# chintha/U-VIP-SLAM

Measured on AMD Instinct MI355X. Metric: frames/sec ORB extract+match, 640x512 @1000 kp, higher is better.
Workload: dtype u8; 1 GPU; BASELINE.json configs[2]: 1xMI355X per rank, batch=256 synthetic 640x512 mono frames (+1 halo frame: the neighbouring rank's first), 1000 feats, 8 levels, fastTh 20, FullDetect extract + all-pairs 256-bit Hamming knn-2 of consecutive frames, HBM-resident I/O; batch_per_gpu=256, pipeline_depth=2, input_batches_in_rotation=4, fast_mode=adaptive

## Files before the change

### u-vip-slam_amd/csrc/hamming.hip

```cpp
#include "common.hpp"

namespace uvo {

constexpr int HM_TILE = 128;

__device__ __forceinline__ int popc256(const uint4& qa, const uint4& qb, const uint4& ta, const uint4& tb) {
  int d = __popc(qa.x ^ ta.x);
  d += __popc(qa.y ^ ta.y);
  d += __popc(qa.z ^ ta.z);
  d += __popc(qa.w ^ ta.w);
  d += __popc(qb.x ^ tb.x);
  d += __popc(qb.y ^ tb.y);
  d += __popc(qb.z ^ tb.z);
  d += __popc(qb.w ^ tb.w);
  return d;
}

__device__ __forceinline__ int clamp_count(int n, int cap) { return n < 0 ? 0 : (n > cap ? cap : n); }

__global__ __launch_bounds__(256) void k_knn2(const uint8_t* __restrict__ q, const int32_t* __restrict__ nq_arr, int nq_fixed, int q_stride,
                                              const uint8_t* __restrict__ t, const int32_t* __restrict__ nt_arr, int nt_fixed, int t_stride,
                                              const uint8_t* __restrict__ mask, int out_stride, int32_t* __restrict__ idx0,
                                              uint16_t* __restrict__ d0, int32_t* __restrict__ idx1, uint16_t* __restrict__ d1) {
  __shared__ uint4 s_t[HM_TILE * 2];
  const int pair = blockIdx.y;
  const int nq = nq_arr ? clamp_count(nq_arr[pair], q_stride < out_stride ? q_stride : out_stride) : nq_fixed;
  const int nt = nt_arr ? clamp_count(nt_arr[pair], t_stride < 65535 ? t_stride : 65535) : nt_fixed;
  const int qi = blockIdx.x * 256 + threadIdx.x;
  if (blockIdx.x * 256 >= nq) return;
  const uint4* Q = reinterpret_cast<const uint4*>(q + (int64_t)pair * q_stride * 32);
  const uint4* T = reinterpret_cast<const uint4*>(t + (int64_t)pair * t_stride * 32);
  const bool live = qi < nq;
  uint4 qa = make_uint4(0, 0, 0, 0), qb = qa;
  if (live) {
    qa = Q[2 * qi];
    qb = Q[2 * qi + 1];
  }
  uint32_t k0 = 0xFFFFFFFFu, k1 = 0xFFFFFFFFu;
  const uint8_t* mrow = mask ? mask + (int64_t)qi * nt : nullptr;
  for (int base = 0; base < nt; base += HM_TILE) {
    const int cnt = nt - base < HM_TILE ? nt - base : HM_TILE;
    __syncthreads();
    if ((int)threadIdx.x < 2 * cnt) s_t[threadIdx.x] = T[2 * base + threadIdx.x];
    __syncthreads();
    if (live) {
      for (int j = 0; j < cnt; ++j) {
        const uint32_t d = (uint32_t)popc256(qa, qb, s_t[2 * j], s_t[2 * j + 1]);
        uint32_t key = (d << 16) | (uint32_t)(base + j);
        if (mrow && !mrow[base + j]) key = 0xFFFFFFFFu;
        const uint32_t lo = min(k0, key);
        k1 = min(k1, max(k0, key));
        k0 = lo;
      }
    }
  }
  if (live) {
    const int64_t o = (int64_t)pair * out_stride + qi;
    idx0[o] = k0 == 0xFFFFFFFFu ? -1 : (int32_t)(k0 & 0xffffu);
    d0[o] = k0 == 0xFFFFFFFFu ? (uint16_t)0xFFFF : (uint16_t)(k0 >> 16);
    idx1[o] = k1 == 0xFFFFFFFFu ? -1 : (int32_t)(k1 & 0xffffu);
    d1[o] = k1 == 0xFFFFFFFFu ? (uint16_t)0xFFFF : (uint16_t)(k1 >> 16);
  }
}

typedef int v4i __attribute__((ext_vector_type(4)));
typedef int v16i __attribute__((ext_vector_type(16)));
constexpr int KM_ROW = 272;

__device__ __forceinline__ uint32_t spread4(uint32_t t) { return (__umul24(t & 0xfu, 0x00204081u)) & 0x01010101u; }
__device__ __forceinline__ v4i spread16(uint32_t x) {
  v4i r;
  r.x = (int)spread4(x), r.y = (int)spread4(x >> 4), r.z = (int)spread4(x >> 8), r.w = (int)spread4(x >> 12);
  return r;
}
__device__ __forceinline__ uint32_t spread4_ff(uint32_t t) {
  const uint32_t b = spread4(t);
  return (b << 8) - b;
}
__device__ __forceinline__ v4i spread16_ff(uint32_t x) {
  v4i r;
  r.x = (int)spread4_ff(x), r.y = (int)spread4_ff(x >> 4), r.z = (int)spread4_ff(x >> 8), r.w = (int)spread4_ff(x >> 12);
  return r;
}

__device__ __forceinline__ int med3_i32(int a, int b, int c) {
  int r;
  asm("v_med3_i32 %0, %1, %2, %3" : "=v"(r) : "v"(a), "v"(b), "v"(c));
  return r;
}

#ifndef UVO_OCC_KNN
#define UVO_OCC_KNN 6
#endif
__global__ __launch_bounds__(256, UVO_OCC_KNN) void k_knn2_mfma(const uint8_t* __restrict__ q, const int32_t* __restrict__ nq_arr, int nq_fixed, int q_stride,
                                                   const uint8_t* __restrict__ t, const int32_t* __restrict__ nt_arr, int nt_fixed, int t_stride,
                                                   int out_stride, int32_t* __restrict__ idx0, uint16_t* __restrict__ d0,
                                                   int32_t* __restrict__ idx1, uint16_t* __restrict__ d1) {
  __shared__ __attribute__((aligned(16))) uint8_t s_exp[32 * KM_ROW];
  __shared__ __attribute__((aligned(16))) int32_t s_key[32];
  const int pair = blockIdx.y;
  const int nq = nq_arr ? clamp_count(nq_arr[pair], q_stride < out_stride ? q_stride : out_stride) : nq_fixed;
  const int nt = nt_arr ? clamp_count(nt_arr[pair], t_stride < 65535 ? t_stride : 65535) : nt_fixed;
  if (blockIdx.x * 128 >= nq) return;
  const int lane = threadIdx.x & 63, wv = wave_in_block();
  const int r = lane & 31, h = lane >> 5;
  const int qi = blockIdx.x * 128 + wv * 32 + r;
  const uint32_t* Q = reinterpret_cast<const uint32_t*>(q + (int64_t)pair * q_stride * 32);
  const uint32_t* T = reinterpret_cast<const uint32_t*>(t + (int64_t)pair * t_stride * 32);
  v4i bq[8];
  int popq = 0;
#pragma unroll
  for (int s = 0; s < 8; ++s) {
    const uint32_t w = qi < nq ? Q[(int64_t)qi * 8 + s] : 0u;
    popq += __popc(w);
    bq[s] = spread16_ff(w >> (16 * h));
  }
  int k0 = 0x7fffffff, k1 = 0x7fffffff;
  const int erow = threadIdx.x >> 3, ec = threadIdx.x & 7;
  uint32_t wnext = erow < nt ? T[(int64_t)erow * 8 + ec] : 0u;
  for (int base = 0; base < nt; base += 32) {
    __syncthreads();
    {
      const int tr = base + erow;
      const uint32_t w = wnext;
      wnext = tr + 32 < nt ? T[(int64_t)(tr + 32) * 8 + ec] : 0u;
      v4i* dst = reinterpret_cast<v4i*>(s_exp + erow * KM_ROW + ec * 32);
      dst[0] = spread16(w), dst[1] = spread16(w >> 16);
      int pc = __popc(w);
      pc += __shfl_xor(pc, 1, 64);
      pc += __shfl_xor(pc, 2, 64);
      pc += __shfl_xor(pc, 4, 64);
      if (ec == 0) s_key[erow] = tr < nt ? ((pc << 16) | tr) : 0x7fff0000;
    }
    __syncthreads();
    v16i acc = {0, 0, 0, 0, 0, 0, 0, 0, 0, 0, 0, 0, 0, 0, 0, 0};
    const uint8_t* arow = s_exp + r * KM_ROW + 16 * h;
#pragma unroll
    for (int s = 0; s < 8; ++s) {
      const v4i a = *reinterpret_cast<const v4i*>(arow + 32 * s);
      acc = __builtin_amdgcn_mfma_i32_32x32x32_i8(a, bq[s], acc, 0, 0, 0);
    }
#pragma unroll
    for (int g = 0; g < 4; ++g) {
      const v4i kb = *reinterpret_cast<const v4i*>(&s_key[8 * g + 4 * h]);
      const int kbv[4] = {kb.x, kb.y, kb.z, kb.w};
#pragma unroll
      for (int e = 0; e < 4; ++e) {
        const int key = (int)(((uint32_t)acc[4 * g + e] << 17) + (uint32_t)kbv[e]);
        k1 = med3_i32(k0, k1, key);
        k0 = min(k0, key);
      }
    }
  }
  const int o0 = __shfl_xor(k0, 32, 64), o1 = __shfl_xor(k1, 32, 64);
  const int m0 = min(k0, o0), m1 = min(max(k0, o0), min(k1, o1));
  if (h == 0 && qi < nq) {
    const int64_t o = (int64_t)pair * out_stride + qi;
    const bool v0 = m0 < 0x7fff0000, v1 = m1 < 0x7fff0000;
    idx0[o] = v0 ? (m0 & 0xffff) : -1;
    d0[o] = v0 ? (uint16_t)((m0 >> 16) + popq) : (uint16_t)0xFFFF;
    idx1[o] = v1 ? (m1 & 0xffff) : -1;
    d1[o] = v1 ? (uint16_t)((m1 >> 16) + popq) : (uint16_t)0xFFFF;
  }
}

__global__ __launch_bounds__(256) void k_matrix(const uint8_t* __restrict__ q, int nq, const uint8_t* __restrict__ t, int nt,
                                                uint16_t* __restrict__ dist) {
  __shared__ uint4 s_t[HM_TILE * 2];
  const int qi = blockIdx.x * 256 + threadIdx.x;
  const uint4* Q = reinterpret_cast<const uint4*>(q);
  const uint4* T = reinterpret_cast<const uint4*>(t);
  const bool live = qi < nq;
  uint4 qa = make_uint4(0, 0, 0, 0), qb = qa;
  if (live) {
    qa = Q[2 * qi];
    qb = Q[2 * qi + 1];
  }
  const int base = blockIdx.y * HM_TILE;
  const int cnt = nt - base < HM_TILE ? nt - base : HM_TILE;
  if ((int)threadIdx.x < 2 * cnt) s_t[threadIdx.x] = T[2 * base + threadIdx.x];
  __syncthreads();
  if (!live) return;
  for (int j = 0; j < cnt; ++j) dist[(int64_t)qi * nt + base + j] = (uint16_t)popc256(qa, qb, s_t[2 * j], s_t[2 * j + 1]);
}

__global__ __launch_bounds__(256) void k_medoid(const uint8_t* __restrict__ desc, const int32_t* __restrict__ offsets, int32_t* __restrict__ best_idx,
                                                int32_t* __restrict__ best_median) {
  __shared__ uint32_t s_best;
  const int p = blockIdx.x;
  const int o0 = offsets[p], n = offsets[p + 1] - o0;
  if (threadIdx.x == 0) s_best = 0xFFFFFFFFu;
  __syncthreads();
  if (n > 0) {
    const uint4* D = reinterpret_cast<const uint4*>(desc + (int64_t)o0 * 32);
    const int k = (int)(0.5 * (n - 1));
    for (int i = threadIdx.x; i < n; i += 256) {
      const uint4 qa = D[2 * i], qb = D[2 * i + 1];
      int lo = 0, hi = 256;
      while (lo < hi) {
        const int mid = (lo + hi) >> 1;
        int c = 0;
        for (int j = 0; j < n; ++j) c += popc256(qa, qb, D[2 * j], D[2 * j + 1]) <= mid;
        if (c >= k + 1)
          hi = mid;
        else
          lo = mid + 1;
      }
      atomicMin(&s_best, ((uint32_t)lo << 16) | (uint32_t)i);
    }
  }
  __syncthreads();
  if (threadIdx.x == 0) {
    best_idx[p] = n > 0 ? (int32_t)(s_best & 0xffffu) : -1;
    best_median[p] = n > 0 ? (int32_t)(s_best >> 16) : -1;
  }
}

void launch_medoid(hipStream_t s, const uint8_t* d_desc, const int32_t* d_offsets, int npoints, int32_t* d_idx, int32_t* d_med) {
  hipLaunchKernelGGL(k_medoid, dim3(npoints), dim3(256), 0, s, d_desc, d_offsets, d_idx, d_med);
}

void launch_knn2(hipStream_t s, int pairs, int max_q, const uint8_t* d_q, const int32_t* d_nq, int nq_fixed, int q_stride, const uint8_t* d_t,
                 const int32_t* d_nt, int nt_fixed, int t_stride, const uint8_t* d_mask, int out_stride, int32_t* d_idx0, uint16_t* d_d0,
                 int32_t* d_idx1, uint16_t* d_d1) {
  if (!d_mask) {
    hipLaunchKernelGGL(k_knn2_mfma, dim3((max_q + 127) / 128, pairs), dim3(256), 0, s, d_q, d_nq, nq_fixed, q_stride, d_t, d_nt, nt_fixed, t_stride,
                       out_stride, d_idx0, d_d0, d_idx1, d_d1);
    return;
  }
  hipLaunchKernelGGL(k_knn2, dim3((max_q + 255) / 256, pairs), dim3(256), 0, s, d_q, d_nq, nq_fixed, q_stride, d_t, d_nt, nt_fixed, t_stride,
                     d_mask, out_stride, d_idx0, d_d0, d_idx1, d_d1);
}

void launch_matrix(hipStream_t s, const uint8_t* d_q, int nq, const uint8_t* d_t, int nt, uint16_t* d_dist) {
  hipLaunchKernelGGL(k_matrix, dim3((nq + 255) / 256, (nt + HM_TILE - 1) / HM_TILE), dim3(256), 0, s, d_q, nq, d_t, nt, d_dist);
}

}
```

### u-vip-slam_amd/csrc/tune_internal.h

```cpp
#pragma once
#define UVO_TUNE_PYR_RING 12
#define UVO_TUNE_FUSE_BLUR_TREE 10
#define UVO_TUNE_PYR_FORM 13
#define UVO_PYR_FORM_AUTO 0
#define UVO_PYR_FORM_LEVELS 1
#define UVO_PYR_FORM_TILES 2
#define UVO_PYR_FORM_ROWS 3
#define UVO_TUNE_PYR_TILE_GROUP 14
#define UVO_TUNE_FEW_FRAMES 16
#define UVO_TUNE_ZERO_COPY_OUT 17
#define UVO_TUNE_SPIN_WAIT 18
```

### u-vip-slam_amd/csrc/gauss_body.hpp

```cpp
#pragma once
#include "common.hpp"
#include "fast_geom.hpp"
#include <type_traits>

namespace uvo {

typedef unsigned short u16x2 __attribute__((ext_vector_type(2)));
__device__ __forceinline__ u16x2 pk(uint32_t x) { return __builtin_bit_cast(u16x2, x); }

struct GaussRowTaps {
  uint32_t l0, c0, l1, c1, r1, l2, c2, r2, c3, r3;
};
__device__ __forceinline__ GaussRowTaps gauss_row_taps(int4 t) {
  auto pk4 = [](int a, int b, int c, int d) { return (uint32_t)a | ((uint32_t)b << 8) | ((uint32_t)c << 16) | ((uint32_t)d << 24); };
  GaussRowTaps T;
  T.l0 = pk4(0, t.x, t.y, t.z), T.c0 = pk4(t.w, t.z, t.y, t.x);
  T.l1 = pk4(0, 0, t.x, t.y), T.c1 = pk4(t.z, t.w, t.z, t.y), T.r1 = pk4(t.x, 0, 0, 0);
  T.l2 = pk4(0, 0, 0, t.x), T.c2 = pk4(t.y, t.z, t.w, t.z), T.r2 = pk4(t.y, t.x, 0, 0);
  T.c3 = pk4(t.x, t.y, t.z, t.w), T.r3 = pk4(t.z, t.y, t.x, 0);
  return T;
}
__device__ __forceinline__ void gauss_row_pass(uint32_t L, uint32_t C, uint32_t R, const GaussRowTaps& T, float* h) {
  const uint32_t s0 = __builtin_amdgcn_udot4(C, T.c0, __builtin_amdgcn_udot4(L, T.l0, 0u, false), false);
  const uint32_t s1 = __builtin_amdgcn_udot4(R, T.r1, __builtin_amdgcn_udot4(C, T.c1, __builtin_amdgcn_udot4(L, T.l1, 0u, false), false), false);
  const uint32_t s2 = __builtin_amdgcn_udot4(R, T.r2, __builtin_amdgcn_udot4(C, T.c2, __builtin_amdgcn_udot4(L, T.l2, 0u, false), false), false);
  const uint32_t s3 = __builtin_amdgcn_udot4(R, T.r3, __builtin_amdgcn_udot4(C, T.c3, 0u, false), false);
  h[0] = (float)s0, h[1] = (float)s1, h[2] = (float)s2, h[3] = (float)s3;
}

struct GaussPlans {
  StripPlan p[kMaxLevels];
};
int gauss7_rows_per_seg(int batch);
int gauss7_blocks_per_frame(const Geom& g, int rows_per_seg);
GaussPlans gauss7_plans(const Geom& g, int rows_per_seg);
constexpr int GS_TILES = 16;
constexpr int GS_TILE_DW = GS_TILES * 32 + 96;
constexpr int GS_LDS_BYTES = 4 * GS_TILE_DW * 4;
template <bool SSE2>
__device__ __forceinline__ void gauss7_body(int block, int blocks_x, int batch, uint32_t (*s_tile)[GS_TILE_DW], const uint8_t* __restrict__ pyr,
                                            uint8_t* __restrict__ blur, int64_t pyr_block, const LevelGeom* __restrict__ lv, int nlevels, int4 taps, int rows_per_seg,
                                            Level0View l0, const GaussPlans& plans) {
  const int vb = xcd_contiguous(block, blocks_x * batch);
  const int vbx = vb % blocks_x, f = vb / blocks_x;
  int item = vbx * 4 + wave_in_block();
  const int lane = threadIdx.x & 63;
  int level = 0;
  for (;; ++level) {
    if (item < plans.p[level].items) break;
    item -= plans.p[level].items;
    if (level == nlevels - 1) return;
  }
  const StripPlan plan = plans.p[level];
  const LevelGeom g = lv[level];
  int strip_x, seg, nsub;
  fast_strip_item(plan, item, strip_x, seg, nsub);
  auto walk = [&](auto ip_tag, auto tail_tag) {
  constexpr bool IP = decltype(ip_tag)::value;
  constexpr bool TAIL = decltype(tail_tag)::value;
  const uint8_t* src = IP ? l0.vbase + f * l0.frame_stride + (int64_t)kPad * l0.pitch + kPad : pyr + f * pyr_block + g.plane_off;
  const int spitch = IP ? l0.pitch : g.pitch;
  uint8_t* dst = blur + f * pyr_block + g.plane_off;

  const int lps = 64 / nsub, sub = (lane * nsub) >> 6, ls = lane - sub * lps;
  const int X = 8 + strip_x + ls * 4;
  int Xc = X > g.pitch - 4 ? g.pitch - 4 : X;
  uint32_t csel = 0x03020100u;
  if (IP) {
    const int x = X - kPad;
    int run = x;
    if (x < 0) run = -x - 3, csel = 0x00010203u;
    else if (x > g.w - 4) run = 2 * (g.w - 1) - x - 3, csel = 0x00010203u;
    Xc = run < 0 ? 0 : (run > g.w - 4 ? g.w - 4 : run);
  }
  const int py0 = 12 + seg * rows_per_seg;
  const int py0l = py0 + sub * rows_per_seg;
  const int py1l = min(py0l + rows_per_seg, g.h + 20);
  const bool lane_out = ls >= 1 && ls <= lps - 2 && X >= 12 && X < g.w + 20 && py1l > py0l;
  const int tile_col = (X >> 4) * 128 + (X & 15);
  const int64_t tile_row_bytes = (int64_t)g.pitch * 8;
  const int x_lo = max(12, 8 + strip_x + 4), x_hi = min(g.w + 20, 8 + strip_x + 4 * (lps - 1));
  const int t_first = (x_lo + 15) >> 4, nts = max((x_hi >> 4) - t_first, 0);
  const int ts_shift = nsub == 1 ? 4 : (nsub == 2 ? 3 : 2), TS = 1 << ts_shift;
  const bool via_lds = lane_out && (X >> 4) >= t_first && (X >> 4) < t_first + nts;
  uint32_t* stile = s_tile[wave_in_block()];
  const int lds_slot = via_lds ? ((sub * TS + ((X >> 4) - t_first)) << 5) + ((X & 15) >> 2) : GS_TILES * 32 + lane;
  const int64_t seg_tile_rows = (int64_t)(rows_per_seg >> 3) * tile_row_bytes;
  const int64_t lane_goff = (int64_t)sub * seg_tile_rows + tile_col;
  int f_lds[2], f_p0[2], f_p1[2], f_rowoff[2];
  int64_t f_goff[2];
#pragma unroll
  for (int it = 0; it < 2; ++it) {
    const int t = lane + 64 * it, row = t & 7, slot = t >> 3, s_ = slot >> ts_shift, ti = slot & (TS - 1);
    const int p0 = py0 + s_ * rows_per_seg;
    f_lds[it] = (slot << 5) + (row << 2);
    f_goff[it] = (int64_t)s_ * seg_tile_rows + (t_first + ti) * 128 + (row << 4);
    f_rowoff[it] = s_ * rows_per_seg + row;
    f_p0[it] = p0, f_p1[it] = (s_ < nsub && ti < nts) ? min(p0 + rows_per_seg, g.h + 20) : p0;
  }
  auto flush_tiles = [&](int pyg, int r_hi, int64_t group_base) {
    __builtin_amdgcn_wave_barrier();
#pragma unroll
    for (int it = 0; it < 2; ++it) {
      const int prow = pyg + f_rowoff[it];
      if ((lane & 7) <= r_hi && prow >= f_p0[it] && prow < f_p1[it]) {
        const uint4 v = *reinterpret_cast<const uint4*>(stile + f_lds[it]);
        *reinterpret_cast<uint4*>(dst + (group_base + f_goff[it])) = v;
      }
    }
    __builtin_amdgcn_wave_barrier();
  };

  const bool tail_lane = SSE2 && (g.w & 3) != 0 && (X - kPad) == (g.w & ~3);
  uint32_t inmask = 0;
#pragma unroll
  for (int k = 0; k < 4; ++k) inmask |= (X + k >= kPad && X + k < g.w + kPad) ? 0xffu << (8 * k) : 0u;
  const int nsrc = min(py0 + rows_per_seg, g.h + 20) - py0 + 6;
  const uint32_t j_in0 = (uint32_t)(kPad - py0l + 6), n_in = (uint32_t)g.h;
  const uint32_t j_edge1 = (lane_out && !via_lds) ? (uint32_t)max(py1l - py0l + 6, 0) : 0u;

  const GaussRowTaps RT = gauss_row_taps(taps);
  const float c0 = (float)taps.x * (1.0f / 65536.0f), c1 = (float)taps.y * (1.0f / 65536.0f), c2 = (float)taps.z * (1.0f / 65536.0f),
              c3 = (float)taps.w * (1.0f / 65536.0f);
  if (!SSE2) __builtin_amdgcn_s_setreg(0x801, 3);
  const int lane_up = (lane > 0 ? lane - 1 : lane) * 4, lane_down = (lane < 63 ? lane + 1 : lane) * 4;
  float hring[7][4];
  uint32_t cring[7];
  auto load_row = [&](int j) -> uint32_t {
    int prow = py0l - 3 + j;
    if (IP) {
      int r = prow - kPad;
      r = r < 0 ? -r : r;
      r = r > g.h - 1 ? 2 * (g.h - 1) - r : r;
      r = r < 0 ? 0 : r;
      const uint32_t v = *reinterpret_cast<const uint32_t*>(src + (__umul24((uint32_t)r, (uint32_t)spitch) + (uint32_t)Xc));
      return __builtin_amdgcn_perm(v, v, csel);
    }
    prow = prow > g.ph - 1 ? g.ph - 1 : prow;
    return *reinterpret_cast<const uint32_t*>(src + (__umul24((uint32_t)prow, (uint32_t)spitch) + (uint32_t)Xc));
  };
  int64_t rowb = (int64_t)(py0 >> 3) * tile_row_bytes + ((py0 & 7) << 4);
  int phase = (py0 - 6) & 7;
  uint32_t cur[7], nxt[7];
#pragma unroll
  for (int u = 0; u < 7; ++u) cur[u] = load_row(u);
  for (int base = 0; base < nsrc; base += 7) {
#pragma unroll
    for (int u = 0; u < 7; ++u) nxt[u] = load_row(base + 7 + u);
#pragma unroll
    for (int u = 0; u < 7; ++u) {
      const int j = base + u;
      if (j < nsrc) {
        const uint32_t C = cur[u];
        const uint32_t L = (uint32_t)__builtin_amdgcn_ds_bpermute(lane_up, (int)C);
        const uint32_t R = (uint32_t)__builtin_amdgcn_ds_bpermute(lane_down, (int)C);
        gauss_row_pass(L, C, R, RT, hring[u]);
        cring[u] = C;
        const int phase_now = phase;
        phase = (phase + 1) & 7;
        if (j >= 6) {
          const float* r0 = hring[(u + 1) % 7];
          const float* r1 = hring[(u + 2) % 7];
          const float* r2 = hring[(u + 3) % 7];
          const float* r3 = hring[(u + 4) % 7];
          const float* r4 = hring[(u + 5) % 7];
          const float* r5 = hring[(u + 6) % 7];
          const float* r6 = hring[u];
          const uint32_t centre = cring[(u + 4) % 7];
          const bool row_in = (uint32_t)j - j_in0 < n_in;
          uint32_t blurred = 0;
#pragma unroll
          for (int k = 0; k < 4; ++k) {
            float z = __builtin_fmaf(c0, r0[k] + r6[k], __builtin_fmaf(c1, r1[k] + r5[k], __builtin_fmaf(c2, r2[k] + r4[k], __builtin_fmaf(c3, r3[k], SSE2 ? 0.0f : 0.5f))));
            if (SSE2 && TAIL) z = tail_lane ? __builtin_floorf(z + 0.5f) : z;
            blurred = __builtin_amdgcn_cvt_pk_u8_f32(z, (uint32_t)k, blurred);
          }
          const uint32_t m = row_in ? inmask : 0u;
          const uint32_t out = (blurred & m) | (centre & ~m);
          stile[lds_slot + (phase_now << 2)] = out;
          if ((uint32_t)j < j_edge1) *reinterpret_cast<uint32_t*>(dst + rowb + lane_goff) = out;
          if (phase_now == 7) {
            flush_tiles(py0 + j - 6 - 7, 7, rowb - 112);
            rowb += tile_row_bytes - 112;
          } else {
            rowb += 16;
          }
        }
      }
    }
#pragma unroll
    for (int u = 0; u < 7; ++u) cur[u] = nxt[u];
  }
  {
    const int py_last = py0 + nsrc - 7;
    if ((py_last & 7) != 7) flush_tiles(py_last & ~7, py_last & 7, (int64_t)(py_last >> 3) * tile_row_bytes);
  }
  };
  const int x_last = 8 + strip_x + 4 * (64 / nsub - 1);
  const bool tail_wave = SSE2 && (g.w & 3) != 0 && kPad + (g.w & ~3) >= 8 + strip_x && kPad + (g.w & ~3) < x_last;
  if (level == 0 && l0.vbase != nullptr)
    walk(std::true_type{}, std::false_type{});
  else if (tail_wave)
    walk(std::false_type{}, std::true_type{});
  else
    walk(std::false_type{}, std::false_type{});
}


}
```

Before: 329,300 frames/s.

## Fold train popcount and index key into MFMA accumulator init for knn2

Reworks the MFMA Hamming knn-2 kernel. When the train count fits in 12 bits, descriptor bits are pre-shifted (<<7 for queries, <<6 for train) so the int8 MFMA directly produces distance<<13 plus the (popcount<<12|index) key loaded as the accumulator init, removing the per-element shift/add. It also widens the workgroup to 8 waves (256 queries) with 64 train rows staged per sync, and uses DPP instead of shuffles for the popcount reduction. Gains are fewer VALU ops and syncs per tile, at the cost of higher register pressure, a second kernel variant for large train sets, and idle non-expander waves during staging.

```diff
diff --git a/u-vip-slam_amd/csrc/hamming.hip b/u-vip-slam_amd/csrc/hamming.hip
--- a/u-vip-slam_amd/csrc/hamming.hip
+++ b/u-vip-slam_amd/csrc/hamming.hip
@@ -1,4 +1,5 @@
 #include "common.hpp"
+#include "tune_internal.h"
 
 namespace uvo {
 
@@ -82,6 +83,25 @@
   r.x = (int)spread4_ff(x), r.y = (int)spread4_ff(x >> 4), r.z = (int)spread4_ff(x >> 8), r.w = (int)spread4_ff(x >> 12);
   return r;
 }
+template <int SH>
+__device__ __forceinline__ uint32_t spread4_at(uint32_t t) {
+  static_assert(SH + 24 < 32, "the product leaves 32 bits");
+  return (__umul24(t & (0xfu << SH), 0x00204081u)) & (0x01010101u << SH);
+}
+template <int SH>
+__device__ __forceinline__ v4i spread16_shl(uint32_t x) {
+  const uint32_t y = x << SH;
+  v4i r;
+  r.x = (int)spread4_at<SH>(y), r.y = (int)spread4_at<SH>(y >> 4), r.z = (int)spread4_at<SH>(y >> 8), r.w = (int)spread4_at<SH>(y >> 12);
+  return r;
+}
+
+__device__ __forceinline__ int sum8_dpp(int v) {
+  v += __builtin_amdgcn_update_dpp(0, v, 0xB1, 0xf, 0xf, true);
+  v += __builtin_amdgcn_update_dpp(0, v, 0x4E, 0xf, 0xf, true);
+  v += __builtin_amdgcn_update_dpp(0, v, 0x141, 0xf, 0xf, true);
+  return v;
+}
 
 __device__ __forceinline__ int med3_i32(int a, int b, int c) {
   int r;
@@ -89,22 +109,33 @@
   return r;
 }
 
-#ifndef UVO_OCC_KNN
-#define UVO_OCC_KNN 6
+#ifndef UVO_KNN_WAVES
+#define UVO_KNN_WAVES 8
 #endif
-__global__ __launch_bounds__(256, UVO_OCC_KNN) void k_knn2_mfma(const uint8_t* __restrict__ q, const int32_t* __restrict__ nq_arr, int nq_fixed, int q_stride,
-                                                   const uint8_t* __restrict__ t, const int32_t* __restrict__ nt_arr, int nt_fixed, int t_stride,
-                                                   int out_stride, int32_t* __restrict__ idx0, uint16_t* __restrict__ d0,
-                                                   int32_t* __restrict__ idx1, uint16_t* __restrict__ d1) {
-  __shared__ __attribute__((aligned(16))) uint8_t s_exp[32 * KM_ROW];
-  __shared__ __attribute__((aligned(16))) int32_t s_key[32];
+#ifndef UVO_KNN_ROWS
+#define UVO_KNN_ROWS 64
+#endif
+constexpr int KM_WAVES = UVO_KNN_WAVES, KM_QUERIES = 32 * KM_WAVES, KM_ROWS = UVO_KNN_ROWS;
+constexpr int KM_FOLD_BITS = 12, KM_FOLD_MAX_TRAIN = 1 << KM_FOLD_BITS;
+static_assert(24 % KM_WAVES == 0 && (KM_ROWS == 32 || KM_ROWS == 64) && KM_ROWS * 8 <= 64 * KM_WAVES, "workgroup shape");
+
+template <bool FOLD>
+__device__ __forceinline__ void knn2_mfma_body(const uint8_t* __restrict__ q, const int32_t* __restrict__ nq_arr, int nq_fixed, int q_stride,
+                                               const uint8_t* __restrict__ t, const int32_t* __restrict__ nt_arr, int nt_fixed, int t_stride,
+                                               int out_stride, int32_t* __restrict__ idx0, uint16_t* __restrict__ d0,
+                                               int32_t* __restrict__ idx1, uint16_t* __restrict__ d1) {
+  __shared__ __attribute__((aligned(16))) uint8_t s_exp[KM_ROWS * KM_ROW];
+  __shared__ __attribute__((aligned(16))) int32_t s_key[KM_ROWS];
+  constexpr int IDX_BITS = FOLD ? KM_FOLD_BITS : 16;
   const int pair = blockIdx.y;
   const int nq = nq_arr ? clamp_count(nq_arr[pair], q_stride < out_stride ? q_stride : out_stride) : nq_fixed;
   const int nt = nt_arr ? clamp_count(nt_arr[pair], t_stride < 65535 ? t_stride : 65535) : nt_fixed;
-  if (blockIdx.x * 128 >= nq) return;
+  if (blockIdx.x * KM_QUERIES >= nq) return;
   const int lane = threadIdx.x & 63, wv = wave_in_block();
   const int r = lane & 31, h = lane >> 5;
-  const int qi = blockIdx.x * 128 + wv * 32 + r;
+  const int qi = blockIdx.x * KM_QUERIES + wv * 32 + r;
+  const bool active = blockIdx.x * KM_QUERIES + wv * 32 < nq;
+  const bool expander = wv < KM_ROWS / 8;
   const uint32_t* Q = reinterpret_cast<const uint32_t*>(q + (int64_t)pair * q_stride * 32);
   const uint32_t* T = reinterpret_cast<const uint32_t*>(t + (int64_t)pair * t_stride * 32);
   v4i bq[8];
@@ -113,42 +144,50 @@
   for (int s = 0; s < 8; ++s) {
     const uint32_t w = qi < nq ? Q[(int64_t)qi * 8 + s] : 0u;
     popq += __popc(w);
-    bq[s] = spread16_ff(w >> (16 * h));
+    bq[s] = FOLD ? spread16_shl<7>(w >> (16 * h)) : spread16_ff(w >> (16 * h));
   }
   int k0 = 0x7fffffff, k1 = 0x7fffffff;
   const int erow = threadIdx.x >> 3, ec = threadIdx.x & 7;
-  uint32_t wnext = erow < nt ? T[(int64_t)erow * 8 + ec] : 0u;
-  for (int base = 0; base < nt; base += 32) {
+  uint32_t wnext = expander && erow < nt ? T[(int64_t)erow * 8 + ec] : 0u;
+  for (int base = 0; base < nt; base += KM_ROWS) {
     __syncthreads();
-    {
+    if (expander) {
       const int tr = base + erow;
       const uint32_t w = wnext;
-      wnext = tr + 32 < nt ? T[(int64_t)(tr + 32) * 8 + ec] : 0u;
+      wnext = tr + KM_ROWS < nt ? T[(int64_t)(tr + KM_ROWS) * 8 + ec] : 0u;
       v4i* dst = reinterpret_cast<v4i*>(s_exp + erow * KM_ROW + ec * 32);
-      dst[0] = spread16(w), dst[1] = spread16(w >> 16);
-      int pc = __popc(w);
-      pc += __shfl_xor(pc, 1, 64);
-      pc += __shfl_xor(pc, 2, 64);
-      pc += __shfl_xor(pc, 4, 64);
-      if (ec == 0) s_key[erow] = tr < nt ? ((pc << 16) | tr) : 0x7fff0000;
+      dst[0] = FOLD ? spread16_shl<6>(w) : spread16(w), dst[1] = FOLD ? spread16_shl<6>(w >> 16) : spread16(w >> 16);
+      const int pc = sum8_dpp(__popc(w));
+      if (ec == 0) s_key[erow] = tr < nt ? ((pc << IDX_BITS) | tr) : 0x7fff0000;
     }
     __syncthreads();
-    v16i acc = {0, 0, 0, 0, 0, 0, 0, 0, 0, 0, 0, 0, 0, 0, 0, 0};
-    const uint8_t* arow = s_exp + r * KM_ROW + 16 * h;
-#pragma unroll
-    for (int s = 0; s < 8; ++s) {
-      const v4i a = *reinterpret_cast<const v4i*>(arow + 32 * s);
-      acc = __builtin_amdgcn_mfma_i32_32x32x32_i8(a, bq[s], acc, 0, 0, 0);
-    }
-#pragma unroll
-    for (int g = 0; g < 4; ++g) {
-      const v4i kb = *reinterpret_cast<const v4i*>(&s_key[8 * g + 4 * h]);
-      const int kbv[4] = {kb.x, kb.y, kb.z, kb.w};
-#pragma unroll
-      for (int e = 0; e < 4; ++e) {
-        const int key = (int)(((uint32_t)acc[4 * g + e] << 17) + (uint32_t)kbv[e]);
-        k1 = med3_i32(k0, k1, key);
-        k0 = min(k0, key);
+    if (active) {
+#pragma unroll
+      for (int sub = 0; sub < KM_ROWS; sub += 32) {
+        if (sub && base + sub >= nt) break;
+        v16i acc;
+#pragma unroll
+        for (int g = 0; g < 4; ++g) {
+          const v4i kb = FOLD ? *reinterpret_cast<const v4i*>(&s_key[sub + 8 * g + 4 * h]) : v4i{0, 0, 0, 0};
+          acc[4 * g] = kb.x, acc[4 * g + 1] = kb.y, acc[4 * g + 2] = kb.z, acc[4 * g + 3] = kb.w;
+        }
+        const uint8_t* arow = s_exp + (sub + r) * KM_ROW + 16 * h;
+#pragma unroll
+        for (int s = 0; s < 8; ++s) {
+          const v4i a = *reinterpret_cast<const v4i*>(arow + 32 * s);
+          acc = __builtin_amdgcn_mfma_i32_32x32x32_i8(a, bq[s], acc, 0, 0, 0);
+        }
+#pragma unroll
+        for (int g = 0; g < 4; ++g) {
+          const v4i kb = FOLD ? v4i{0, 0, 0, 0} : *reinterpret_cast<const v4i*>(&s_key[sub + 8 * g + 4 * h]);
+          const int kbv[4] = {kb.x, kb.y, kb.z, kb.w};
+#pragma unroll
+          for (int e = 0; e < 4; ++e) {
+            const int key = FOLD ? acc[4 * g + e] : (int)(((uint32_t)acc[4 * g + e] << 17) + (uint32_t)kbv[e]);
+            k1 = (FOLD && g == 0 && e == 0) ? min(k1, max(k0, key)) : med3_i32(k0, k1, key);
+            k0 = min(k0, key);
+          }
+        }
       }
     }
   }
@@ -157,11 +196,26 @@
   if (h == 0 && qi < nq) {
     const int64_t o = (int64_t)pair * out_stride + qi;
     const bool v0 = m0 < 0x7fff0000, v1 = m1 < 0x7fff0000;
-    idx0[o] = v0 ? (m0 & 0xffff) : -1;
-    d0[o] = v0 ? (uint16_t)((m0 >> 16) + popq) : (uint16_t)0xFFFF;
-    idx1[o] = v1 ? (m1 & 0xffff) : -1;
-    d1[o] = v1 ? (uint16_t)((m1 >> 16) + popq) : (uint16_t)0xFFFF;
-  }
+    constexpr int IDX_MASK = (1 << IDX_BITS) - 1;
+    idx0[o] = v0 ? (m0 & IDX_MASK) : -1;
+    d0[o] = v0 ? (uint16_t)((m0 >> IDX_BITS) + popq) : (uint16_t)0xFFFF;
+    idx1[o] = v1 ? (m1 & IDX_MASK) : -1;
+    d1[o] = v1 ? (uint16_t)((m1 >> IDX_BITS) + popq) : (uint16_t)0xFFFF;
+  }
+}
+
+#define UVO_KNN2_MFMA_ATTR __attribute__((amdgpu_flat_work_group_size(64 * KM_WAVES, 64 * KM_WAVES), amdgpu_waves_per_eu(6, 6)))
+__global__ UVO_KNN2_MFMA_ATTR void k_knn2_mfma(const uint8_t* __restrict__ q, const int32_t* __restrict__ nq_arr, int nq_fixed, int q_stride,
+                                               const uint8_t* __restrict__ t, const int32_t* __restrict__ nt_arr, int nt_fixed, int t_stride,
+                                               int out_stride, int32_t* __restrict__ idx0, uint16_t* __restrict__ d0,
+                                               int32_t* __restrict__ idx1, uint16_t* __restrict__ d1) {
+  knn2_mfma_body<true>(q, nq_arr, nq_fixed, q_stride, t, nt_arr, nt_fixed, t_stride, out_stride, idx0, d0, idx1, d1);
+}
+__global__ UVO_KNN2_MFMA_ATTR void k_knn2_mfma_wide(const uint8_t* __restrict__ q, const int32_t* __restrict__ nq_arr, int nq_fixed, int q_stride,
+                                                    const uint8_t* __restrict__ t, const int32_t* __restrict__ nt_arr, int nt_fixed, int t_stride,
+                                                    int out_stride, int32_t* __restrict__ idx0, uint16_t* __restrict__ d0,
+                                                    int32_t* __restrict__ idx1, uint16_t* __restrict__ d1) {
+  knn2_mfma_body<false>(q, nq_arr, nq_fixed, q_stride, t, nt_arr, nt_fixed, t_stride, out_stride, idx0, d0, idx1, d1);
 }
 
 __global__ __launch_bounds__(256) void k_matrix(const uint8_t* __restrict__ q, int nq, const uint8_t* __restrict__ t, int nt,
@@ -220,12 +274,20 @@
   hipLaunchKernelGGL(k_medoid, dim3(npoints), dim3(256), 0, s, d_desc, d_offsets, d_idx, d_med);
 }
 
+int knn2_index_bits(int nt_bound) { return nt_bound <= KM_FOLD_MAX_TRAIN ? KM_FOLD_BITS : 16; }
+
 void launch_knn2(hipStream_t s, int pairs, int max_q, const uint8_t* d_q, const int32_t* d_nq, int nq_fixed, int q_stride, const uint8_t* d_t,
                  const int32_t* d_nt, int nt_fixed, int t_stride, const uint8_t* d_mask, int out_stride, int32_t* d_idx0, uint16_t* d_d0,
                  int32_t* d_idx1, uint16_t* d_d1) {
   if (!d_mask) {
-    hipLaunchKernelGGL(k_knn2_mfma, dim3((max_q + 127) / 128, pairs), dim3(256), 0, s, d_q, d_nq, nq_fixed, q_stride, d_t, d_nt, nt_fixed, t_stride,
-                       out_stride, d_idx0, d_d0, d_idx1, d_d1);
+    const int nt_bound = d_nt ? (t_stride < 65535 ? t_stride : 65535) : nt_fixed;
+    const dim3 grid((max_q + KM_QUERIES - 1) / KM_QUERIES, pairs), block(64 * KM_WAVES);
+    if (knn2_index_bits(nt_bound) == KM_FOLD_BITS)
+      hipLaunchKernelGGL(k_knn2_mfma, grid, block, 0, s, d_q, d_nq, nq_fixed, q_stride, d_t, d_nt, nt_fixed, t_stride, out_stride, d_idx0, d_d0,
+                         d_idx1, d_d1);
+    else
+      hipLaunchKernelGGL(k_knn2_mfma_wide, grid, block, 0, s, d_q, d_nq, nq_fixed, q_stride, d_t, d_nt, nt_fixed, t_stride, out_stride, d_idx0,
+                         d_d0, d_idx1, d_d1);
     return;
   }
   hipLaunchKernelGGL(k_knn2, dim3((max_q + 255) / 256, pairs), dim3(256), 0, s, d_q, d_nq, nq_fixed, q_stride, d_t, d_nt, nt_fixed, t_stride,
@@ -237,3 +299,5 @@
 }
 
 }
+
+extern "C" int uvo_knn2_index_bits(int nt_bound) { return uvo::knn2_index_bits(nt_bound); }
diff --git a/u-vip-slam_amd/csrc/tune_internal.h b/u-vip-slam_amd/csrc/tune_internal.h
--- a/u-vip-slam_amd/csrc/tune_internal.h
+++ b/u-vip-slam_amd/csrc/tune_internal.h
@@ -10,3 +10,8 @@
 #define UVO_TUNE_FEW_FRAMES 16
 #define UVO_TUNE_ZERO_COPY_OUT 17
 #define UVO_TUNE_SPIN_WAIT 18
+
+#ifdef __cplusplus
+extern "C"
+#endif
+int uvo_knn2_index_bits(int nt_bound);
```

After: 329,200 frames/s. No clear change (-0.0%).

## Specialize gauss7 walk for single-subsegment waves and simplify address arithmetic

Applied to the files above, without the earlier changes.

Adds a FULL template specialization for waves with nsub==1, which folds away the per-lane subsegment math. It replaces 64-bit address offsets with 32-bit ones and precomputes the flush row bounds so each flush does one comparison. Row loads are now computed per block of seven, with a fast interior path that avoids reflection and clamping. An optional packed-FMA column path is added but stays disabled by default. The extra instantiations grow code size, and the 32-bit offsets assume each plane fits in 4 GB.

```diff
diff --git a/u-vip-slam_amd/csrc/gauss_body.hpp b/u-vip-slam_amd/csrc/gauss_body.hpp
--- a/u-vip-slam_amd/csrc/gauss_body.hpp
+++ b/u-vip-slam_amd/csrc/gauss_body.hpp
@@ -34,6 +34,10 @@
 int gauss7_rows_per_seg(int batch);
 int gauss7_blocks_per_frame(const Geom& g, int rows_per_seg);
 GaussPlans gauss7_plans(const Geom& g, int rows_per_seg);
+#ifndef UVO_GAUSS_PK_COLUMN
+#define UVO_GAUSS_PK_COLUMN 0
+#endif
+typedef float f32x2 __attribute__((ext_vector_type(2)));
 constexpr int GS_TILES = 16;
 constexpr int GS_TILE_DW = GS_TILES * 32 + 96;
 constexpr int GS_LDS_BYTES = 4 * GS_TILE_DW * 4;
@@ -46,23 +50,25 @@
   int item = vbx * 4 + wave_in_block();
   const int lane = threadIdx.x & 63;
   int level = 0;
-  for (;; ++level) {
-    if (item < plans.p[level].items) break;
-    item -= plans.p[level].items;
-    if (level == nlevels - 1) return;
-  }
-  const StripPlan plan = plans.p[level];
+  for (; level < nlevels; ++level) {
+    const int n = plans.p[level].items;
+    if (item < n) break;
+    item -= n;
+  }
+  if (level == nlevels) return;
+  const StripPlan& plan = plans.p[level];
   const LevelGeom g = lv[level];
   int strip_x, seg, nsub;
   fast_strip_item(plan, item, strip_x, seg, nsub);
-  auto walk = [&](auto ip_tag, auto tail_tag) {
+  auto walk = [&](auto ip_tag, auto tail_tag, auto full_tag) {
   constexpr bool IP = decltype(ip_tag)::value;
   constexpr bool TAIL = decltype(tail_tag)::value;
+  constexpr bool FULL = decltype(full_tag)::value;
   const uint8_t* src = IP ? l0.vbase + f * l0.frame_stride + (int64_t)kPad * l0.pitch + kPad : pyr + f * pyr_block + g.plane_off;
   const int spitch = IP ? l0.pitch : g.pitch;
   uint8_t* dst = blur + f * pyr_block + g.plane_off;
 
-  const int lps = 64 / nsub, sub = (lane * nsub) >> 6, ls = lane - sub * lps;
+  const int lps = FULL ? 64 : 64 / nsub, sub = FULL ? 0 : (lane * nsub) >> 6, ls = lane - sub * lps;
   const int X = 8 + strip_x + ls * 4;
   int Xc = X > g.pitch - 4 ? g.pitch - 4 : X;
   uint32_t csel = 0x03020100u;
@@ -74,36 +80,36 @@
     Xc = run < 0 ? 0 : (run > g.w - 4 ? g.w - 4 : run);
   }
   const int py0 = 12 + seg * rows_per_seg;
-  const int py0l = py0 + sub * rows_per_seg;
+  const int sub_rows = sub * rows_per_seg;
+  const int py0l = py0 + sub_rows;
   const int py1l = min(py0l + rows_per_seg, g.h + 20);
   const bool lane_out = ls >= 1 && ls <= lps - 2 && X >= 12 && X < g.w + 20 && py1l > py0l;
-  const int tile_col = (X >> 4) * 128 + (X & 15);
-  const int64_t tile_row_bytes = (int64_t)g.pitch * 8;
+  const uint32_t tile_col = (uint32_t)((X >> 4) * 128 + (X & 15));
+  const uint32_t tile_row_bytes = (uint32_t)g.pitch * 8u;
   const int x_lo = max(12, 8 + strip_x + 4), x_hi = min(g.w + 20, 8 + strip_x + 4 * (lps - 1));
   const int t_first = (x_lo + 15) >> 4, nts = max((x_hi >> 4) - t_first, 0);
-  const int ts_shift = nsub == 1 ? 4 : (nsub == 2 ? 3 : 2), TS = 1 << ts_shift;
+  const int ts_shift = (FULL || nsub == 1) ? 4 : (nsub == 2 ? 3 : 2), TS = 1 << ts_shift;
   const bool via_lds = lane_out && (X >> 4) >= t_first && (X >> 4) < t_first + nts;
   uint32_t* stile = s_tile[wave_in_block()];
   const int lds_slot = via_lds ? ((sub * TS + ((X >> 4) - t_first)) << 5) + ((X & 15) >> 2) : GS_TILES * 32 + lane;
-  const int64_t seg_tile_rows = (int64_t)(rows_per_seg >> 3) * tile_row_bytes;
-  const int64_t lane_goff = (int64_t)sub * seg_tile_rows + tile_col;
-  int f_lds[2], f_p0[2], f_p1[2], f_rowoff[2];
-  int64_t f_goff[2];
+  const uint32_t seg_tile_rows = (uint32_t)(rows_per_seg >> 3) * tile_row_bytes;
+  const uint32_t lane_goff = (uint32_t)sub * seg_tile_rows + tile_col;
+  int f_lds[2], f_lo[2], f_hi[2];
+  uint32_t f_goff[2];
 #pragma unroll
   for (int it = 0; it < 2; ++it) {
     const int t = lane + 64 * it, row = t & 7, slot = t >> 3, s_ = slot >> ts_shift, ti = slot & (TS - 1);
     const int p0 = py0 + s_ * rows_per_seg;
+    const int p1 = (s_ < nsub && ti < nts) ? min(p0 + rows_per_seg, g.h + 20) : p0;
     f_lds[it] = (slot << 5) + (row << 2);
-    f_goff[it] = (int64_t)s_ * seg_tile_rows + (t_first + ti) * 128 + (row << 4);
-    f_rowoff[it] = s_ * rows_per_seg + row;
-    f_p0[it] = p0, f_p1[it] = (s_ < nsub && ti < nts) ? min(p0 + rows_per_seg, g.h + 20) : p0;
-  }
-  auto flush_tiles = [&](int pyg, int r_hi, int64_t group_base) {
+    f_goff[it] = (uint32_t)s_ * seg_tile_rows + (uint32_t)((t_first + ti) * 128 + (row << 4));
+    f_lo[it] = p0 - (s_ * rows_per_seg + row), f_hi[it] = p1 - (s_ * rows_per_seg + row);
+  }
+  auto flush_tiles = [&](int pyg, int r_hi, uint32_t group_base) {
     __builtin_amdgcn_wave_barrier();
 #pragma unroll
     for (int it = 0; it < 2; ++it) {
-      const int prow = pyg + f_rowoff[it];
-      if ((lane & 7) <= r_hi && prow >= f_p0[it] && prow < f_p1[it]) {
+      if ((lane & 7) <= r_hi && pyg >= f_lo[it] && pyg < f_hi[it]) {
         const uint4 v = *reinterpret_cast<const uint4*>(stile + f_lds[it]);
         *reinterpret_cast<uint4*>(dst + (group_base + f_goff[it])) = v;
       }
@@ -116,8 +122,10 @@
 #pragma unroll
   for (int k = 0; k < 4; ++k) inmask |= (X + k >= kPad && X + k < g.w + kPad) ? 0xffu << (8 * k) : 0u;
   const int nsrc = min(py0 + rows_per_seg, g.h + 20) - py0 + 6;
-  const uint32_t j_in0 = (uint32_t)(kPad - py0l + 6), n_in = (uint32_t)g.h;
-  const uint32_t j_edge1 = (lane_out && !via_lds) ? (uint32_t)max(py1l - py0l + 6, 0) : 0u;
+  const uint32_t j_in0s = (uint32_t)(kPad - py0 + 6), n_in = (uint32_t)g.h;
+  const uint32_t j_in0 = j_in0s - (uint32_t)sub_rows;
+  const bool direct_lane = lane_out && !via_lds;
+  const uint32_t j_edge1 = direct_lane ? (uint32_t)max(py1l - py0l + 6, 0) : 0u;
 
   const GaussRowTaps RT = gauss_row_taps(taps);
   const float c0 = (float)taps.x * (1.0f / 65536.0f), c1 = (float)taps.y * (1.0f / 65536.0f), c2 = (float)taps.z * (1.0f / 65536.0f),
@@ -126,27 +134,43 @@
   const int lane_up = (lane > 0 ? lane - 1 : lane) * 4, lane_down = (lane < 63 ? lane + 1 : lane) * 4;
   float hring[7][4];
   uint32_t cring[7];
-  auto load_row = [&](int j) -> uint32_t {
-    int prow = py0l - 3 + j;
+  const uint32_t lane_src = (uint32_t)sub_rows * (uint32_t)spitch + (uint32_t)Xc;
+  const int sub_rows_max = FULL ? 0 : (nsub - 1) * rows_per_seg;
+  auto edge_row = [&](int p) -> uint32_t {
     if (IP) {
-      int r = prow - kPad;
-      r = r < 0 ? -r : r;
+      int r = p < 0 ? -p : p;
       r = r > g.h - 1 ? 2 * (g.h - 1) - r : r;
-      r = r < 0 ? 0 : r;
-      const uint32_t v = *reinterpret_cast<const uint32_t*>(src + (__umul24((uint32_t)r, (uint32_t)spitch) + (uint32_t)Xc));
-      return __builtin_amdgcn_perm(v, v, csel);
-    }
-    prow = prow > g.ph - 1 ? g.ph - 1 : prow;
-    return *reinterpret_cast<const uint32_t*>(src + (__umul24((uint32_t)prow, (uint32_t)spitch) + (uint32_t)Xc));
-  };
-  int64_t rowb = (int64_t)(py0 >> 3) * tile_row_bytes + ((py0 & 7) << 4);
+      return (uint32_t)(r < 0 ? 0 : r);
+    }
+    return (uint32_t)(p > g.ph - 1 ? g.ph - 1 : p);
+  };
+  auto load_block = [&](int j0, uint32_t* rows) {
+    const int p_first = py0 - 3 + j0 - (IP ? kPad : 0), p_last = p_first + 6 + sub_rows_max;
+    const bool inside = p_first >= 0 && p_last <= (IP ? g.h : g.ph) - 1;
+    uint32_t off[7];
+    if (inside) {
+      const uint32_t o = (uint32_t)p_first * (uint32_t)spitch;
+#pragma unroll
+      for (int u = 0; u < 7; ++u) off[u] = (o + (uint32_t)(u * spitch)) + lane_src;
+    } else if (FULL) {
+#pragma unroll
+      for (int u = 0; u < 7; ++u) off[u] = edge_row(p_first + u) * (uint32_t)spitch + (uint32_t)Xc;
+    } else {
+#pragma unroll
+      for (int u = 0; u < 7; ++u) off[u] = __umul24(edge_row(p_first + u + sub_rows), (uint32_t)spitch) + (uint32_t)Xc;
+    }
+#pragma unroll
+    for (int u = 0; u < 7; ++u) {
+      const uint32_t v = *reinterpret_cast<const uint32_t*>(src + off[u]);
+      rows[u] = IP ? __builtin_amdgcn_perm(v, v, csel) : v;
+    }
+  };
+  uint32_t rowb = (uint32_t)(py0 >> 3) * tile_row_bytes + (uint32_t)((py0 & 7) << 4);
   int phase = (py0 - 6) & 7;
   uint32_t cur[7], nxt[7];
-#pragma unroll
-  for (int u = 0; u < 7; ++u) cur[u] = load_row(u);
+  load_block(0, cur);
   for (int base = 0; base < nsrc; base += 7) {
-#pragma unroll
-    for (int u = 0; u < 7; ++u) nxt[u] = load_row(base + 7 + u);
+    load_block(base + 7, nxt);
 #pragma unroll
     for (int u = 0; u < 7; ++u) {
       const int j = base + u;
@@ -167,18 +191,34 @@
           const float* r5 = hring[(u + 6) % 7];
           const float* r6 = hring[u];
           const uint32_t centre = cring[(u + 4) % 7];
-          const bool row_in = (uint32_t)j - j_in0 < n_in;
+          const bool row_in = (uint32_t)j - (FULL ? j_in0s : j_in0) < n_in;
           uint32_t blurred = 0;
+#if UVO_GAUSS_PK_COLUMN
+#pragma unroll
+          for (int kp = 0; kp < 4; kp += 2) {
+            auto pr = [&](const float* r) { return f32x2{r[kp], r[kp + 1]}; };
+            const f32x2 bias = SSE2 ? f32x2{0.0f, 0.0f} : f32x2{0.5f, 0.5f};
+            const f32x2 z2 = __builtin_elementwise_fma(f32x2{c0, c0}, pr(r0) + pr(r6), __builtin_elementwise_fma(f32x2{c1, c1}, pr(r1) + pr(r5),
+                                 __builtin_elementwise_fma(f32x2{c2, c2}, pr(r2) + pr(r4), __builtin_elementwise_fma(f32x2{c3, c3}, pr(r3), bias))));
+#pragma unroll
+            for (int e = 0; e < 2; ++e) {
+              float z = z2[e];
+              if (SSE2 && TAIL) z = tail_lane ? __builtin_floorf(z + 0.5f) : z;
+              blurred = __builtin_amdgcn_cvt_pk_u8_f32(z, (uint32_t)(kp + e), blurred);
+            }
+          }
+#else
 #pragma unroll
           for (int k = 0; k < 4; ++k) {
             float z = __builtin_fmaf(c0, r0[k] + r6[k], __builtin_fmaf(c1, r1[k] + r5[k], __builtin_fmaf(c2, r2[k] + r4[k], __builtin_fmaf(c3, r3[k], SSE2 ? 0.0f : 0.5f))));
             if (SSE2 && TAIL) z = tail_lane ? __builtin_floorf(z + 0.5f) : z;
             blurred = __builtin_amdgcn_cvt_pk_u8_f32(z, (uint32_t)k, blurred);
           }
+#endif
           const uint32_t m = row_in ? inmask : 0u;
           const uint32_t out = (blurred & m) | (centre & ~m);
           stile[lds_slot + (phase_now << 2)] = out;
-          if ((uint32_t)j < j_edge1) *reinterpret_cast<uint32_t*>(dst + rowb + lane_goff) = out;
+          if (FULL ? direct_lane : (uint32_t)j < j_edge1) *reinterpret_cast<uint32_t*>(dst + (rowb + lane_goff)) = out;
           if (phase_now == 7) {
             flush_tiles(py0 + j - 6 - 7, 7, rowb - 112);
             rowb += tile_row_bytes - 112;
@@ -193,18 +233,22 @@
   }
   {
     const int py_last = py0 + nsrc - 7;
-    if ((py_last & 7) != 7) flush_tiles(py_last & ~7, py_last & 7, (int64_t)(py_last >> 3) * tile_row_bytes);
+    if ((py_last & 7) != 7) flush_tiles(py_last & ~7, py_last & 7, (uint32_t)(py_last >> 3) * tile_row_bytes);
   }
   };
   const int x_last = 8 + strip_x + 4 * (64 / nsub - 1);
   const bool tail_wave = SSE2 && (g.w & 3) != 0 && kPad + (g.w & ~3) >= 8 + strip_x && kPad + (g.w & ~3) < x_last;
-  if (level == 0 && l0.vbase != nullptr)
-    walk(std::true_type{}, std::false_type{});
-  else if (tail_wave)
-    walk(std::false_type{}, std::true_type{});
-  else
-    walk(std::false_type{}, std::false_type{});
-}
-
-
-}
+  const bool in_place = level == 0 && l0.vbase != nullptr;
+  if (tail_wave && !in_place)
+    walk(std::false_type{}, std::true_type{}, std::false_type{});
+  else if (nsub == 1) {
+    if (in_place) walk(std::true_type{}, std::false_type{}, std::true_type{});
+    else walk(std::false_type{}, std::false_type{}, std::true_type{});
+  } else {
+    if (in_place) walk(std::true_type{}, std::false_type{}, std::false_type{});
+    else walk(std::false_type{}, std::false_type{}, std::false_type{});
+  }
+}
+
+
+}
```

Measured after the change: 321,500 frames/s before, 327,700 frames/s after (median of 6 runs). 1.9% higher.
